# ligeroinc/ligero-prover

Measured on AMD Instinct MI355X. Metric: prover constraints/sec, higher is better.
Workload: dtype u32 limbs (BN254 Fr: 256-bit modular integers, 9x29-bit limbs in registers; SHA-256 words)

## Files before the change

### ligero-prover_amd/csrc/aes.hip

```cpp
#include "fr29.hpp"
#include "kernels.hpp"
#include <cstdlib>

namespace lig {

namespace {
struct AesTables { uint32_t te0[256]; uint8_t sbox[256]; };

uint8_t xtime_h(uint8_t x) { return (uint8_t)((x << 1) ^ ((x >> 7) * 0x1b)); }

const AesTables& host_tables() {
    static AesTables T;
    static bool ready = false;
    if (!ready) {
        uint8_t p = 1, q = 1;
        do {
            p = (uint8_t)(p ^ (p << 1) ^ ((p & 0x80) ? 0x1b : 0));
            q ^= (uint8_t)(q << 1); q ^= (uint8_t)(q << 2); q ^= (uint8_t)(q << 4);
            if (q & 0x80) q ^= 0x09;
            auto rol = [](uint8_t v, int s) { return (uint8_t)((v << s) | (v >> (8 - s))); };
            T.sbox[p] = (uint8_t)(q ^ rol(q, 1) ^ rol(q, 2) ^ rol(q, 3) ^ rol(q, 4) ^ 0x63);
        } while (p != 1);
        T.sbox[0] = 0x63;
        for (int i = 0; i < 256; i++) {
// ... 9 lines not shown
void aes256_expand_host(const uint8_t key[32], uint32_t rk[60]) {
    const AesTables& T = host_tables();
    auto subw = [&](uint32_t t) {
        return ((uint32_t)T.sbox[t >> 24] << 24) | ((uint32_t)T.sbox[(t >> 16) & 255] << 16) |
               ((uint32_t)T.sbox[(t >> 8) & 255] << 8) | T.sbox[t & 255];
    };
    for (int i = 0; i < 8; i++)
        rk[i] = ((uint32_t)key[4 * i] << 24) | ((uint32_t)key[4 * i + 1] << 16) | ((uint32_t)key[4 * i + 2] << 8) | key[4 * i + 3];
    uint8_t rcon = 1;
    for (int i = 8; i < 60; i++) {
        uint32_t t = rk[i - 1];
        if (i % 8 == 0) { t = subw((t << 8) | (t >> 24)) ^ ((uint32_t)rcon << 24); rcon = xtime_h(rcon); }
        else if (i % 8 == 4) t = subw(t);
        rk[i] = rk[i - 8] ^ t;
    }
}

__device__ uint32_t g_te[4 * 256];

__device__ __forceinline__ uint32_t x3(uint32_t a, uint32_t b, uint32_t c) { return __builtin_amdgcn_bitop3_b32(a, b, c, 0x96); }

struct TeView { const uint32_t* base; uint32_t off; };
template <int LOGR, int LAYOUT>
__device__ __forceinline__ uint32_t te_at(const TeView& tv, uint32_t table, uint32_t word, int shift) {
    if constexpr (LAYOUT == 1) {
        static_assert(LOGR == 4 || LAYOUT == 0, "entry-major layout: 16 replicas");
        const uint32_t a = __builtin_amdgcn_perm(word, tv.off, 0x0c0c0000u | ((4u + (uint32_t)(shift >> 3)) << 8));
        return *reinterpret_cast<const uint32_t*>(reinterpret_cast<const char*>(tv.base) + a + table * 64u);
    } else {
        const uint32_t idx = shift == 24 ? (word >> 24) : ((word >> shift) & 255u);
        return tv.base[((table << 8) + idx) << LOGR];
    }
}
template <int LOGR, int LAYOUT>
__device__ __forceinline__ void aes256_block(const uint32_t* __restrict__ rk, const TeView& tl, uint64_t block_index, uint32_t out[4]) {
    uint32_t s0 = rk[0], s1 = rk[1], s2 = (uint32_t)(block_index >> 32) ^ rk[2], s3 = (uint32_t)block_index ^ rk[3];
#define T_(t, w, sh) te_at<LOGR, LAYOUT>(tl, t, w, sh)
#pragma unroll
    for (int r = 1; r < 14; r++) {
        const uint32_t a0 = x3(T_(0, s0, 24), T_(1, s1, 16), T_(2, s2, 8)), a1 = x3(T_(0, s1, 24), T_(1, s2, 16), T_(2, s3, 8));
        const uint32_t a2 = x3(T_(0, s2, 24), T_(1, s3, 16), T_(2, s0, 8)), a3 = x3(T_(0, s3, 24), T_(1, s0, 16), T_(2, s1, 8));
        const uint32_t b0 = x3(a0, T_(3, s3, 0), rk[4 * r]), b1 = x3(a1, T_(3, s0, 0), rk[4 * r + 1]);
        const uint32_t b2 = x3(a2, T_(3, s1, 0), rk[4 * r + 2]), b3 = x3(a3, T_(3, s2, 0), rk[4 * r + 3]);
        s0 = b0; s1 = b1; s2 = b2; s3 = b3;
    }
    out[0] = x3(T_(2, s0, 24) & 0xff000000u, T_(3, s1, 16) & 0x00ff0000u, T_(0, s2, 8) & 0x0000ff00u) ^ (T_(1, s3, 0) & 0xffu) ^ rk[56];
    out[1] = x3(T_(2, s1, 24) & 0xff000000u, T_(3, s2, 16) & 0x00ff0000u, T_(0, s3, 8) & 0x0000ff00u) ^ (T_(1, s0, 0) & 0xffu) ^ rk[57];
    out[2] = x3(T_(2, s2, 24) & 0xff000000u, T_(3, s3, 16) & 0x00ff0000u, T_(0, s0, 8) & 0x0000ff00u) ^ (T_(1, s1, 0) & 0xffu) ^ rk[58];
    out[3] = x3(T_(2, s3, 24) & 0xff000000u, T_(3, s0, 16) & 0x00ff0000u, T_(0, s1, 8) & 0x0000ff00u) ^ (T_(1, s2, 0) & 0xffu) ^ rk[59];
#undef T_
}
template <int LOGR, int LAYOUT>
__device__ __forceinline__ TeView te_stage(uint32_t* te) {
    if constexpr (LAYOUT == 1) {
        for (uint32_t i = threadIdx.x; i < (1024u << LOGR); i += blockDim.x) te[i] = g_te[(((i >> 4) & 3u) << 8) + (i >> 6)];
        __syncthreads();
        return TeView{te, (threadIdx.x & 15u) * 4u};
    } else {
        for (uint32_t i = threadIdx.x; i < (1024u << LOGR); i += blockDim.x) te[i] = g_te[i >> LOGR];
        __syncthreads();
        return TeView{te + (threadIdx.x & ((1u << LOGR) - 1)), 0u};
    }
}
template <int LOGR, int LAYOUT>
__device__ __forceinline__ fr aes_field_elem(const uint32_t* __restrict__ rk, const TeView& tl, uint64_t elem) {
    uint32_t o[8];
    aes256_block<LOGR, LAYOUT>(rk, tl, 2 * elem, o);
    aes256_block<LOGR, LAYOUT>(rk, tl, 2 * elem + 1, o + 4);
    fr v;
#pragma unroll
    for (int i = 0; i < 8; i++) v.v[i] = __builtin_bswap32(o[i]);
#pragma unroll
    for (int i = 0; i < 8; i++) v.v[i] = (v.v[i] >> 2) | (i < 7 ? (v.v[i + 1] << 30) : 0u);
    return fr_reduce_once(v);
}

template <int LOGR, int LAYOUT = 0>
__global__ void __launch_bounds__(256) k_rng_fill(const uint32_t* __restrict__ rk, uint64_t first_elem, fr* __restrict__ out, size_t count) {
    __shared__ uint32_t te[1024 << LOGR];
    const TeView tl = te_stage<LOGR, LAYOUT>(te);
    for (size_t e = (size_t)blockIdx.x * blockDim.x + threadIdx.x; e < count; e += (size_t)gridDim.x * blockDim.x)
        fr_store(out + e, aes_field_elem<LOGR, LAYOUT>(rk, tl, first_elem + e));
}

template <int LOGR, int LAYOUT = 0>
__global__ void __launch_bounds__(256) k_rng_fill_indexed(const uint32_t* __restrict__ rk, uint64_t first_elem, const uint32_t* __restrict__ idx,
                                                          fr* __restrict__ out, size_t count) {
    __shared__ uint32_t te[1024 << LOGR];
    const TeView tl = te_stage<LOGR, LAYOUT>(te);
    for (size_t e = (size_t)blockIdx.x * blockDim.x + threadIdx.x; e < count; e += (size_t)gridDim.x * blockDim.x)
        fr_store(out + e, aes_field_elem<LOGR, LAYOUT>(rk, tl, first_elem + idx[e]));
}

template <int LOGR, int LAYOUT = 0>
__global__ void __launch_bounds__(256) k_rng_fill_rows(const uint32_t* __restrict__ rk, uint64_t first, fr* __restrict__ out, size_t rows,
                                                       uint32_t per_row, size_t row_stride, uint32_t col_off, uint32_t elem_stride, uint64_t stream_stride) {
    __shared__ uint32_t te[1024 << LOGR];
    const TeView tl = te_stage<LOGR, LAYOUT>(te);
    const size_t total = rows * per_row;
    for (size_t e = (size_t)blockIdx.x * blockDim.x + threadIdx.x; e < total; e += (size_t)gridDim.x * blockDim.x) {
        const size_t r = e / per_row;
        const uint32_t i = (uint32_t)(e - r * per_row);
        fr_store(out + r * row_stride + col_off + (size_t)i * elem_stride, aes_field_elem<LOGR, LAYOUT>(rk, tl, first + r * stream_stride + i));
    }
}
template <int LOGR, int LAYOUT = 0>
__global__ void __launch_bounds__(256) k_rng_fill_rows_dense(const uint32_t* __restrict__ rk, uint64_t first, fr* __restrict__ out, size_t rows,
                                                             uint32_t per_row, uint32_t k) {
    __shared__ uint32_t te[1024 << LOGR];
    const TeView tl = te_stage<LOGR, LAYOUT>(te);
    const size_t total = rows * k;
    for (size_t e = (size_t)blockIdx.x * blockDim.x + threadIdx.x; e < total; e += (size_t)gridDim.x * blockDim.x) {
        const size_t r = e / k;
        const uint32_t i = (uint32_t)(e - r * k);
        fr_store(out + e, i < per_row ? aes_field_elem<LOGR, LAYOUT>(rk, tl, first + r * (uint64_t)per_row + i) : fr_zero());
    }
}
#ifndef LIG_RLC_THREADS
#define LIG_RLC_THREADS 256
#endif
template <int LOGR, int LAYOUT = 0>
__global__ void __launch_bounds__(LIG_RLC_THREADS) k_rand_rlc(const uint32_t* __restrict__ rk, uint64_t first, fr* __restrict__ rand_out,
                                                  const fr* __restrict__ msgs, size_t rows, uint32_t per_row, uint32_t k,
                                                  const f29s* __restrict__ rc, uint32_t group_rows, fr* __restrict__ code_part,
                                                  fr* __restrict__ lin_part) {
    __shared__ uint32_t te[1024 << LOGR];
    const TeView tl = te_stage<LOGR, LAYOUT>(te);
    const uint32_t jblocks = k / blockDim.x, groups = (uint32_t)((rows + group_rows - 1) / group_rows), tiles = jblocks * groups;
    for (uint32_t tile = blockIdx.x; tile < tiles; tile += gridDim.x) {
        const uint32_t g = tile / jblocks, j = (tile - g * jblocks) * blockDim.x + threadIdx.x;
        const size_t r0 = (size_t)g * group_rows, r1 = r0 + group_rows < rows ? r0 + group_rows : rows;
        const bool live = j < per_row;
        f29 ac = rc != nullptr ? unpack29(fr_load(code_part + (size_t)g * k + j)) : f29_zero(), al = f29_zero();
        int since = 0;
        for (size_t r = r0; r < r1; r++) {
            const f29 u = unpack29(fr_load(msgs + r * k + j));
            if (rc != nullptr) ac = f29_add(ac, f29_montmul(u, f29_load_tab(rc + r)));
            fr v = fr_zero();
            if (live) {
                v = aes_field_elem<LOGR, LAYOUT>(rk, tl, first + r * (uint64_t)per_row + j);
                al = f29_add(al, f29_montmul(u, unpack29(v)));
            }
            fr_store(rand_out + r * k + j, v);
            if (++since == 6) { ac = f29_qnorm(ac); al = f29_qnorm(al); since = 0; }
        }
        if (rc != nullptr) fr_store(code_part + (size_t)g * k + j, pack29(f29_reduce_2p(ac)));
        f29 w = f29_montmul(f29_qnorm(al), f29_const_r2());
        w = f29_reduce_2p(f29_add(w, unpack29(fr_load(lin_part + (size_t)g * k + j))));
        fr_store(lin_part + (size_t)g * k + j, pack29(w));
    }
}

static constexpr size_t BIG_FILL = (size_t)1 << 20;
#ifndef LIG_AES_REP
#define LIG_AES_REP 4
#endif
static constexpr int REP = LIG_AES_REP;
static constexpr uint32_t BIG_BLOCKS_MAX = 256u * (REP >= 4 ? 2u : REP == 3 ? 4u : 8u);
#define BIG_BLOCKS (lig::knobs().aes_blocks ? lig::knobs().aes_blocks : BIG_BLOCKS_MAX)
#define PERM_LAYOUT (REP == 4 && lig::knobs().aes_layout == 1)
static inline uint32_t small_blocks(size_t total, size_t cap) { size_t b = (total + 255) / 256; return (uint32_t)(b > cap ? cap : b); }
void launch_rng_fill_rows_dense(hipStream_t s, const uint32_t* rk60_dev, uint64_t first, fr* out, size_t rows, uint32_t per_row, uint32_t k) {
    const size_t total = rows * k;
    if (!total) return;
    if (total >= BIG_FILL && PERM_LAYOUT) hipLaunchKernelGGL((k_rng_fill_rows_dense<4, 1>), dim3(BIG_BLOCKS), dim3(256), 0, s, rk60_dev, first, out, rows, per_row, k);
    else if (total >= BIG_FILL) hipLaunchKernelGGL(k_rng_fill_rows_dense<REP>, dim3(BIG_BLOCKS), dim3(256), 0, s, rk60_dev, first, out, rows, per_row, k);
    else hipLaunchKernelGGL(k_rng_fill_rows_dense<0>, dim3(small_blocks(total, 8192)), dim3(256), 0, s, rk60_dev, first, out, rows, per_row, k);
}

void launch_rand_rlc(hipStream_t s, const uint32_t* rk60_dev, uint64_t first, fr* out, const fr* msgs, size_t rows, uint32_t per_row, uint32_t k,
                     const f29s* rc_dev, uint32_t group_rows, fr* code_part, fr* lin_part) {
    if (!rows) return;
    const uint32_t th = (k % LIG_RLC_THREADS == 0) ? LIG_RLC_THREADS : 256;
    const size_t tiles = (size_t)(k / th) * ((rows + group_rows - 1) / group_rows);
    if (rows * k >= BIG_FILL && PERM_LAYOUT)
        hipLaunchKernelGGL((k_rand_rlc<4, 1>), dim3((uint32_t)(tiles < BIG_BLOCKS ? tiles : BIG_BLOCKS)), dim3(th), 0, s, rk60_dev, first, out, msgs, rows, per_row, k,
                           rc_dev, group_rows, code_part, lin_part);
    else if (rows * k >= BIG_FILL)
        hipLaunchKernelGGL(k_rand_rlc<REP>, dim3((uint32_t)(tiles < BIG_BLOCKS ? tiles : BIG_BLOCKS)), dim3(th), 0, s, rk60_dev, first, out, msgs, rows, per_row, k,
                           rc_dev, group_rows, code_part, lin_part);
    else
        hipLaunchKernelGGL(k_rand_rlc<0>, dim3((uint32_t)(tiles < 8192 ? tiles : 8192)), dim3(th), 0, s, rk60_dev, first, out, msgs, rows, per_row, k, rc_dev,
                           group_rows, code_part, lin_part);
}

void launch_rng_fill_rows(hipStream_t s, const uint32_t* rk60_dev, uint64_t first, fr* out, size_t rows, uint32_t per_row,
                          size_t row_stride, uint32_t col_off, uint32_t elem_stride, uint64_t stream_stride) {
    const size_t total = rows * per_row;
    if (!total) return;
    if (total >= BIG_FILL && PERM_LAYOUT)
        hipLaunchKernelGGL((k_rng_fill_rows<4, 1>), dim3(BIG_BLOCKS), dim3(256), 0, s, rk60_dev, first, out, rows, per_row, row_stride, col_off, elem_stride, stream_stride);
    else if (total >= BIG_FILL)
        hipLaunchKernelGGL(k_rng_fill_rows<REP>, dim3(BIG_BLOCKS), dim3(256), 0, s, rk60_dev, first, out, rows, per_row, row_stride, col_off, elem_stride, stream_stride);
    else
        hipLaunchKernelGGL(k_rng_fill_rows<0>, dim3(small_blocks(total, 8192)), dim3(256), 0, s, rk60_dev, first, out, rows, per_row, row_stride, col_off,
                           elem_stride, stream_stride);
}

void aes_upload_tables() {
    const AesTables& T = host_tables();
    uint32_t te[4 * 256];
    for (int t = 0; t < 4; t++)
        for (int i = 0; i < 256; i++) te[256 * t + i] = t ? (T.te0[i] >> (8 * t)) | (T.te0[i] << (32 - 8 * t)) : T.te0[i];
    (void)hipMemcpyToSymbol(HIP_SYMBOL(g_te), te, sizeof(te));
}

void launch_rng_fill(hipStream_t s, const uint32_t* rk60_dev, uint64_t first_elem, fr* out, size_t count) {
    if (!count) return;
    if (count >= BIG_FILL && PERM_LAYOUT) hipLaunchKernelGGL((k_rng_fill<4, 1>), dim3(BIG_BLOCKS), dim3(256), 0, s, rk60_dev, first_elem, out, count);
    else if (count >= BIG_FILL) hipLaunchKernelGGL(k_rng_fill<REP>, dim3(BIG_BLOCKS), dim3(256), 0, s, rk60_dev, first_elem, out, count);
    else hipLaunchKernelGGL(k_rng_fill<0>, dim3(small_blocks(count, 4096)), dim3(256), 0, s, rk60_dev, first_elem, out, count);
}

void launch_rng_fill_indexed(hipStream_t s, const uint32_t* rk60_dev, uint64_t first_elem, const uint32_t* idx_dev, fr* out, size_t count) {
    if (!count) return;
    if (count >= BIG_FILL && PERM_LAYOUT) hipLaunchKernelGGL((k_rng_fill_indexed<4, 1>), dim3(BIG_BLOCKS), dim3(256), 0, s, rk60_dev, first_elem, idx_dev, out, count);
// ... 6 lines not shown
```

### ligero-prover_amd/csrc/ctx_internal.hpp

```cpp
#pragma once
#include <hip/hip_runtime.h>
#include <functional>
#include <mutex>
#include <string>
#include <unordered_map>
#include <utility>
#include <vector>
#include "../../include/lig_hip.h"
#include "kernels.hpp"

using lig::fr;


struct lig_ctx {
    int device = 0;
    uint32_t l = 0, k = 0, n = 0;
    hipStream_t stream = nullptr;
    hipStream_t stream2 = nullptr;
    bool side_shared = false, copy_is_main = false;
    hipStream_t stream3 = nullptr;
    hipStream_t stream_sha = nullptr;
    hipEvent_t ev_fork = nullptr, ev_join = nullptr;
    lig::NttPlan plan_half;
    std::string err;
// ... 15 lines not shown
    uint32_t* tri_dev = nullptr; size_t tri_cap = 0;
    bool streams_shared = false;
    bool prof_on = false;
    std::vector<std::pair<hipEvent_t, hipEvent_t>> prof_events;
    size_t prof_used = 0;
    uint64_t prof_rows = 0;
    std::vector<uint32_t> prof_launch_rows;
    std::vector<std::pair<void*, void (*)(void*)>> comms;
    std::mutex debug_mu;
    std::function<std::string()> debug_state;
};
inline hipStream_t lig_internal_copy_stream(lig_ctx* c) {
    if (!c->stream3 && hipStreamCreateWithFlags(&c->stream3, hipStreamNonBlocking) != hipSuccess) { (void)hipGetLastError(); c->stream3 = c->stream; c->copy_is_main = true; }
    return c->stream3;
}
inline void sync_all_streams(lig_ctx* c) { for (hipStream_t st : {c->stream, c->stream2, c->stream3, c->stream_sha}) if (st) (void)hipStreamSynchronize(st); }
inline void lig_internal_set_debug_state(lig_ctx* c, std::function<std::string()> f) { std::lock_guard<std::mutex> lk(c->debug_mu); c->debug_state = std::move(f); }
inline std::string lig_internal_debug_state(lig_ctx* c) { std::lock_guard<std::mutex> lk(c->debug_mu); return c->debug_state ? c->debug_state() : std::string(); }

inline void lig_internal_comms_release(lig_ctx* c) {
    auto v = std::move(c->comms);
    c->comms.clear();
    for (auto& e : v) e.second(e.first);
}
inline void lig_internal_comm_unregister(lig_ctx* c, void* obj) {
    for (size_t i = 0; i < c->comms.size(); i++) if (c->comms[i].first == obj) { c->comms.erase(c->comms.begin() + i); return; }
}

int lig_internal_comm_fault(lig_ctx* c, bool stream_ordered);

int lig_internal_encode_rows(lig_ctx* c, const void* msgs, void* out, size_t rows, int mode, hipStream_t on = nullptr, int phases = 15,
                             void* y_scratch = nullptr, void* z_scratch = nullptr);
int lig_internal_encode_dot(lig_ctx* c, const void* rands, size_t rows, const void* cw2, size_t cw2_stride, uint32_t group_rows, void* part, hipStream_t on = nullptr,
                            bool cw2_z = false);
int lig_internal_extend_2k(lig_ctx* c, void* buf);
int lig_internal_decode_to(lig_ctx* c, const void* src, void* dst);
int lig_internal_encode_2k_rows(lig_ctx* c, void* buf, size_t rows, hipStream_t on = nullptr);
int lig_internal_encode_generic(lig_ctx* c, void* buf, hipStream_t on = nullptr);
int lig_internal_upload_small(lig_ctx* c, void* dst, const void* src, size_t bytes, hipStream_t st);
int lig_internal_download(lig_ctx* c, void* host_pinned, const void* src, size_t bytes, hipStream_t st);
int lig_internal_reserve_scratch(lig_ctx* c, size_t rows);

#define CHECK_CTX(c) do { if (!(c)) return LIG_E_ARG; if (hipSetDevice((c)->device) != hipSuccess) { (c)->err = "hipSetDevice failed"; return LIG_E_HIP; } } while (0)
#define HIP_TRY(c, call) do { hipError_t e__ = (call); if (e__ != hipSuccess) { (c)->err = std::string(#call) + ": " + hipGetErrorString(e__); return LIG_E_HIP; } } while (0)
#define FAIL(c, code, msg) do { (c)->err = (msg); return (code); } while (0)
```

### ligero-prover_amd/csrc/kernels.hpp

```cpp
#pragma once
#include <hip/hip_runtime.h>
#include <stddef.h>
#include <stdint.h>
#include <string>
#include "fr.hpp"

namespace lig {
struct Knobs {
    int      encode_kmask = 15;
    uint32_t k13_block = 256;
    uint32_t k2_dyn_lds = 0;
    size_t   encode_chunk = 512;
    bool     encode_generic = false;
    uint32_t sha_block = 256;
    int      sha_ws = 2;
    uint32_t aes_blocks = 0;
    bool     shared_side = true;
    int      aes_layout = 1;
    int      sha_gate = 1;
    size_t   sha_gate_rows = 2;
    int      sha_prio = 0;
    int      ctx_low_prio_every = 0;
    int      sha_cumask = 0;
    size_t   s1_head = 128, s1_tail = 96, s2_head = 192;
    bool     fused_rlc = true;
    bool     early_code = true;
    int      upload_mode = 2;
    bool     upload_prio = true;
    int      fault_upload = 0;
    int      upload_timeout_s = 5;
    bool     shard_uploader = false;
    int      rands_upload_mode = 2;
    bool     spin_wait = true;
    int      spin_wait_ms = 50;
    bool     d2h_kernel = true;
    bool     shard_force_exchange = false;
    bool     zres = false;
    bool     trace = false;
    int      fault_comm = 0;
    int      comm_timeout_s = 300;
    int      ipc_host_s = 120;
    int      ipc_stall_s = 120;
    std::string stream_map;
    std::string stream_pad;
    std::string rccl_lib;
};
const Knobs& knobs();
}

namespace lig {

struct NttPlan {
    uint32_t N = 0, log2N = 0;
    fr* w = nullptr;
    fr* winv = nullptr;
    fr ninv;
};
// ... 71 lines not shown
```

### ligero-prover_amd/csrc/lig_capi.hip

```cpp
#include <hip/hip_runtime.h>
#include <atomic>
#include <cstdio>
#include <cstdlib>
#include <cstring>
#include <string>
#include <unordered_map>
#include <vector>

#include <unistd.h>
#include "../../include/lig_hip.h"
#include "host_field.hpp"
#include "kernels.hpp"
#include "fr29.hpp"
#include "ctx_internal.hpp"

namespace lig {
void aes_upload_tables();
void launch_rng_fill_rows_dense(hipStream_t s, const uint32_t* rk60_dev, uint64_t first, fr* out, size_t rows, uint32_t per_row, uint32_t k);
}

namespace H = lig::host;

static fr to_dev(const H::Fr& a) {
    fr r;
// ... 229 lines not shown
            for (uint32_t j = 0; j < M / 2; j++) t[(M / 2 - 1) + j] = to_f29s(pw[(size_t)j * (S / M)]);
        t[S - 1] = to_f29s(H::from_u64(1));
        return t;
    };
    int rc;
    if ((rc = upload29(c, stage_table(H::pow_u64(w, B), A), &tp.tw_a)) != LIG_OK) return rc;
    if ((rc = upload29(c, stage_table(H::pow_u64(w, A), B), &tp.tw_b)) != LIG_OK) return rc;
    std::vector<lig::f29s> mid((size_t)N);
    const H::Fr scale = inverse ? H::inv(H::from_u64(N)) : H::from_u64(1);
    H::Fr base = H::from_u64(1);
    for (uint32_t k1 = 0; k1 < A; k1++) {
        H::Fr cur = scale;
        for (uint32_t n2 = 0; n2 < B; n2++) { mid[(size_t)k1 * B + n2] = to_f29s(cur); cur = H::mul(cur, base); }
        base = H::mul(base, w);
    }
    return upload29(c, mid, &tp.mid);
}

const lig::Knobs& lig::knobs() {
    static const lig::Knobs k = [] {
        lig::Knobs t;
        auto num = [](const char* name, long dflt) { const char* e = std::getenv(name); return e && *e ? std::atol(e) : dflt; };
        auto pos = [&](const char* name, long dflt) { const long v = num(name, 0); return v > 0 ? v : dflt; };
        t.encode_kmask = (int)num("LIG_ENCODE_KMASK", 15);
        { const long v = num("LIG_K13_BLOCK", 0); t.k13_block = (v == 64 || v == 128) ? (uint32_t)v : 256u; }
        t.k2_dyn_lds = (uint32_t)num("LIG_K2_DYN_LDS", 0);
        t.encode_chunk = (size_t)pos("LIG_ENCODE_CHUNK", 512);
        { const char* e = std::getenv("LIG_ENCODE_GENERIC"); t.encode_generic = e && e[0] == '1'; }
        t.sha_block = (uint32_t)pos("LIG_SHA_BLOCK", 256);
        { const long v = num("LIG_SHA_WS", 2); t.sha_ws = (v == 0 || v == 1 || v == 4) ? (int)v : 2; }
        t.sha_gate = (int)num("LIG_SHA_GATE", 1);
        { const long v = num("LIG_AES_BLOCKS", 0); t.aes_blocks = v >= 64 && v <= 4096 ? (uint32_t)v : 0u; }
        t.aes_layout = (int)num("LIG_AES_LAYOUT", 1);
        t.shared_side = num("LIG_SHARED_SIDE", 1) != 0;
        t.sha_gate_rows = (size_t)pos("LIG_SHA_GATE_ROWS", 2);
#ifdef LIG_EXPERIMENTS
        t.sha_prio = (int)num("LIG_SHA_PRIO", 0);
        if (const char* v = std::getenv("LIG_STREAM_MAP")) t.stream_map = v;
        if (const char* v = std::getenv("LIG_STREAM_PAD")) t.stream_pad = v;
        t.sha_cumask = (int)num("LIG_SHA_CUMASK", 0);
        t.ctx_low_prio_every = (int)num("LIG_CTX_LOW_PRIO_EVERY", 0);
#endif
        t.s1_head = (size_t)num("LIG_S1_HEAD", 128); t.s1_tail = (size_t)num("LIG_S1_TAIL", 96); t.s2_head = (size_t)num("LIG_S2_HEAD", 192);
        t.fused_rlc = std::getenv("LIG_NO_FUSED_RLC") == nullptr;
        t.early_code = num("LIG_EARLY_CODE", 1) != 0;
        t.upload_mode = (int)num("LIG_UPLOAD_MODE", 2);
        t.rands_upload_mode = (int)num("LIG_RANDS_UPLOAD_MODE", 2);
        t.upload_prio = num("LIG_UPLOAD_PRIO", 1) != 0;
        t.shard_uploader = num("LIG_SHARD_UPLOADER", 0) != 0;
        t.upload_timeout_s = (int)pos("LIG_UPLOAD_TIMEOUT_S", 5);
        t.fault_upload = (int)num("LIG_FAULT_UPLOAD", 0);
        t.d2h_kernel = num("LIG_D2H_KERNEL", 1) != 0;
        t.spin_wait = num("LIG_SPIN_WAIT", 1) != 0;
        t.spin_wait_ms = (int)pos("LIG_SPIN_WAIT_MS", 50);
        t.shard_force_exchange = std::getenv("LIG_SHARD_FORCE_EXCHANGE") != nullptr;
        t.trace = std::getenv("LIG_TRACE") != nullptr;
        t.zres = num("LIG_ZRES", 0) != 0;
        t.fault_comm = (int)num("LIG_FAULT_COMM", 0);
        t.ipc_stall_s = (int)pos("LIG_IPC_STALL_S", 120);
        t.ipc_host_s = (int)pos("LIG_IPC_HOST_S", 120);
        t.comm_timeout_s = (int)pos("LIG_COMM_TIMEOUT_S", 300);
        { const char* e = std::getenv("LIG_RCCL_LIB"); if (e) t.rccl_lib = e; }
        return t;
    }();
    return k;
}

int lig_internal_comm_fault(lig_ctx* c, bool stream_ordered) {
    const int f = lig::knobs().fault_comm;
    if (!f) return 0;
    if (f == 3 && stream_ordered) for (;;) sleep(3600);
    if ((stream_ordered && (f == 1 || f == 2)) || (!stream_ordered && f == 2)) {
        if (c) c->err = std::string("injected fault (LIG_FAULT_COMM) in the ") + (stream_ordered ? "stream-ordered" : "host-synchronous") + " all-to-all";
        return 1;
    }
// ... 306 lines not shown
            HIP_TRY(c, hipMemcpy2DAsync(z, n * sizeof(fr), (const fr*)msgs + r0 * k, k * sizeof(fr), k * sizeof(fr), nr, hipMemcpyDeviceToDevice, st));
            lig::ntt_generic_inverse(st, c->plan[LIG_SIZE_K], z, nr, n);
            lig::ntt_generic_forward(st, c->plan[LIG_SIZE_N], z, nr, n);
            for (size_t r = 0; r < nr; r++)
                for (uint32_t cs = 1; cs < 4; cs++)
                    HIP_TRY(c, hipMemcpy2DAsync((fr*)out + (r0 + r) * 3 * k + (cs - 1) * k, sizeof(fr), z + r * n + cs, 4 * sizeof(fr), sizeof(fr), k,
                                                hipMemcpyDeviceToDevice, st));
        }
    } else if (!half) {
        HIP_TRY(c, hipMemsetAsync(out, 0, rows * out_stride * sizeof(fr), st));
        HIP_TRY(c, hipMemcpy2DAsync(out, out_stride * sizeof(fr), msgs, (size_t)c->k * sizeof(fr), (size_t)c->k * sizeof(fr),
                                    rows, hipMemcpyDeviceToDevice, st));
        lig::ntt_generic_inverse(st, c->plan[LIG_SIZE_K], (fr*)out, rows, out_stride);
        lig::ntt_generic_forward(st, c->plan[LIG_SIZE_N], (fr*)out, rows, out_stride);
    } else {
        const size_t k2 = 2 * (size_t)c->k, chunk = 64;
        int rc = ensure_scratch(c, rows < chunk ? rows : chunk);
        if (rc != LIG_OK) return rc;
        for (size_t r0 = 0; r0 < rows; r0 += chunk) {
            const size_t nr = rows - r0 < chunk ? rows - r0 : chunk;
            fr* z = c->scratch_z;
            HIP_TRY(c, hipMemsetAsync(z, 0, nr * k2 * sizeof(fr), st));
            HIP_TRY(c, hipMemcpy2DAsync(z, k2 * sizeof(fr), (const fr*)msgs + r0 * c->k, (size_t)c->k * sizeof(fr), (size_t)c->k * sizeof(fr),
                                        nr, hipMemcpyDeviceToDevice, st));
            lig::ntt_generic_inverse(st, c->plan[LIG_SIZE_K], z, nr, k2);
            lig::ntt_generic_forward(st, c->plan_half, z, nr, k2);
            HIP_TRY(c, hipMemcpy2DAsync((fr*)out + r0 * c->k, sizeof(fr), z + 1, 2 * sizeof(fr), sizeof(fr), nr * (size_t)c->k,
                                        hipMemcpyDeviceToDevice, st));
        }
    }
    HIP_TRY(c, hipGetLastError());
    return LIG_OK;
}
int lig_internal_encode_dot(lig_ctx* c, const void* rands, size_t rows, const void* cw2, size_t cw2_stride, uint32_t group_rows, void* part, hipStream_t on, bool cw2_z) {
    if (!c->fast) return LIG_E_STATE;
    hipStream_t st = on ? on : c->stream;
    int rc = ensure_scratch(c, rows);
    if (rc != LIG_OK) return rc;
    const lig::EncodeDot dot{(const fr*)cw2, cw2_stride, group_rows, (fr*)part, cw2_z};
    lig::encode_rows_fast(st, c->ep, (const fr*)rands, nullptr, c->scratch_y, c->scratch_z, rows, nullptr, nullptr, lig::ENC_DOT, &dot);
    HIP_TRY(c, hipGetLastError());
    return LIG_OK;
}
static fr* tiled_scratch_for(lig_ctx* c, hipStream_t st) { return c->tiled_scratch[st == c->stream2 ? 1 : 0]; }

int lig_internal_encode_2k_rows(lig_ctx* c, void* buf, size_t rows, hipStream_t on) {
    hipStream_t st = on ? on : c->stream;
    if (c->tiled && rows <= 3) {
        lig::ntt_tiled(st, c->tplan[LIG_SIZE_2K][1], (fr*)buf, c->n, (fr*)buf, c->n, rows, tiled_scratch_for(c, st));
        lig::ntt_tiled(st, c->tplan[LIG_SIZE_N][0], (fr*)buf, c->n, (fr*)buf, c->n, rows, tiled_scratch_for(c, st));
        HIP_TRY(c, hipGetLastError());
        return LIG_OK;
    }
    lig::ntt_generic_inverse(st, c->plan[LIG_SIZE_2K], (fr*)buf, rows, c->n);
    lig::ntt_generic_forward(st, c->plan[LIG_SIZE_N], (fr*)buf, rows, c->n);
    HIP_TRY(c, hipGetLastError());
    return LIG_OK;
}
int lig_internal_encode_generic(lig_ctx* c, void* buf, hipStream_t on) {
    hipStream_t st = on ? on : c->stream;
    if (c->tiled) {
        lig::ntt_tiled(st, c->tplan[LIG_SIZE_K][1], (fr*)buf, c->n, (fr*)buf, c->n, 1, tiled_scratch_for(c, st));
        lig::ntt_tiled(st, c->tplan[LIG_SIZE_N][0], (fr*)buf, c->n, (fr*)buf, c->n, 1, tiled_scratch_for(c, st));
        HIP_TRY(c, hipGetLastError());
        return LIG_OK;
    }
    lig::ntt_generic_inverse(st, c->plan[LIG_SIZE_K], (fr*)buf, 1, c->n);
    lig::ntt_generic_forward(st, c->plan[LIG_SIZE_N], (fr*)buf, 1, c->n);
    HIP_TRY(c, hipGetLastError());
    return LIG_OK;
}
int lig_internal_decode_to(lig_ctx* c, const void* src, void* dst) {
    if (c->tiled) {
// ... 301 lines not shown
```

### ligero-prover_amd/csrc/prover.hip

```cpp
#include "prover_common.hpp"
#include "upload.hpp"
#include <cerrno>
#include <functional>

struct lig_trace {
    lig_ctx* c = nullptr;
    lig_synth_job job;
    bool from_rows = false;
    bool loaded = false, committed = false;
    bool dense_rands = false;
    bool diag_ok = false;
    fr* msgs_alt = nullptr;
    bool alt_pending = false;
    JobHeader hdr;
    std::vector<RowDesc> rows;
    std::vector<PadRun> pad_runs;
    uint64_t mask_pos = 0;
    std::vector<std::pair<size_t, size_t>> sched1;
    const uint8_t* host_msgs = nullptr;
    std::vector<hipEvent_t> ev_up;
    FlagPage flags;
    UploadLane up, rand;
    bool up_by_thread = false;
    fr* rands_full = nullptr;
// ... 329 lines not shown
struct RandSource { const fr* dev = nullptr; const uint8_t* host = nullptr; bool pushed = false;
                    lig_linear* linear = nullptr; };

static int prove_stage23(lig_trace* T, const RandSource& rs, const uint8_t* const_sum_given, const uint8_t** proof, size_t* proof_len,
                         lig_proof_info* info, const std::function<void(const char*)>& mark) {
    lig_ctx* c = T->c;
    const uint32_t l = c->l, k = c->k, n = c->n, t = 192;
    const size_t R = T->R;
    hipStream_t s = c->stream, s2 = c->stream2;
    auto t0 = clk::now();
    uint32_t rk[60];
    const size_t NT = T->triples.size() / 3;
    lig::aes256_expand_host(info->stage1_seed, rk);
    TRY(lig_internal_upload_small(c, c->rk_dev, rk, sizeof rk, s));
    fr* code = T->acc; fr* lin = T->acc + n; fr* quad = T->acc + 2 * (size_t)n; fr* tmp = T->acc + 3 * (size_t)n;
    fr* linH = lin + 2 * (size_t)k; fr* linC = lin + 3 * (size_t)k;
    const size_t groups = (lig_tune::CHUNK + lig_tune::GROUP - 1) / lig_tune::GROUP;
    fr* p_code = T->parts; fr* p_linH = T->parts + groups * (size_t)n; fr* p_linC = T->parts + 2 * groups * (size_t)n;
    const size_t dot_groups = (lig_tune::CHUNK + lig_tune::DOT_GROUP - 1) / lig_tune::DOT_GROUP;
    HIP_TRY(c, hipMemsetAsync(T->parts, 0, (2 * groups * (size_t)n + dot_groups * k) * 32, s));
    HIP_TRY(c, hipMemsetAsync(T->acc, 0, 4 * (size_t)n * 32, s));
    fr* rhalf = T->rcw;
    const size_t s2_head = lig::knobs().s2_head;
    const std::vector<std::pair<size_t, size_t>> sched2 = chunk_schedule(R, lig_tune::CHUNK, s2_head, 0);
    const size_t n_chunks = sched2.size();
    std::vector<uint64_t> chunk_pos(n_chunks + 1, 0);
    for (size_t ci = 0; ci < n_chunks; ci++) {
        uint64_t cnt = 0;
        for (size_t r = sched2[ci].first; r < sched2[ci].second; r++) cnt += T->rows[r].data;
        chunk_pos[ci + 1] = chunk_pos[ci] + cnt;
    }
    auto rand_buf = [&](size_t ci) -> fr* { return rs.dev ? const_cast<fr*>(rs.dev) + sched2[ci].first * (size_t)k : T->randb + (ci & 1) * lig_tune::CHUNK * (size_t)k; };
    const bool fused_rlc = !rs.dev && !rs.host && (k % 256 == 0) && lig::knobs().fused_rlc;
    const bool early_code = lig::knobs().early_code;
    const lig::f29s* rc_loop = early_code ? nullptr : T->coef_dev;
    const bool rands_by_thread = rs.host && lig::knobs().upload_mode == 2 && lig::knobs().rands_upload_mode == 2 && lig_internal_uploader_available(c) && n_chunks;
    uint32_t rseq = 0;
    const lig::FlagLayout fl = T->flag_layout(n_chunks);
    if (rands_by_thread) {
        TRY(T->flags.ensure(c, fl.words));
        if (fl.consumed + n_chunks > fl.words) FAIL(c, LIG_E_STATE, "rows job: flag page too small for the stage-2 schedule");
        rseq = ++T->rand.seq;
        T->up_abort.store(0, std::memory_order_release);
        std::vector<lig::UploadChunk> chunks;
        for (size_t ci = 0; ci < n_chunks; ci++) chunks.push_back({(uint8_t*)rand_buf(ci), rs.host + sched2[ci].first * (size_t)k * 32, (sched2[ci].second - sched2[ci].first) * (size_t)k * 32});
        lig_internal_uploader_submit(c->device, lig::chunk_jobs(chunks, T->flags.host + fl.rands, rseq, &T->rand.failed, T->flags.host + fl.consumed, &T->up_abort, 1), &T->rand.pending);
    }
    auto form_rand_chunk = [&](size_t ci) -> int {
        const size_t b = sched2[ci].first, nb = sched2[ci].second - sched2[ci].first;
        fr* rb = rand_buf(ci);
        if (rs.pushed) return LIG_OK;
        if (rs.dev) { HIP_TRY(c, hipEventRecord(T->ev_ready[ci & 1], s2)); return LIG_OK; }
        if (rands_by_thread) return LIG_OK;
        if (ci >= 2) HIP_TRY(c, hipStreamWaitEvent(s2, T->ev_used[ci & 1], 0));
        if (rs.host) {
            HIP_TRY(c, hipMemcpyAsync(rb, rs.host + b * (size_t)k * 32, nb * (size_t)k * 32, hipMemcpyHostToDevice, s2));
        } else {
            uint64_t lpos = chunk_pos[ci];
            for (size_t r = 0; r < nb;) {
                size_t run = 1;
                const uint32_t d = T->rows[b + r].data;
                while (r + run < nb && T->rows[b + r + run].data == d) run++;
                if (fused_rlc) lig::launch_rand_rlc(s2, c->rk_dev, lpos, rb + r * k, T->msgs + (b + r) * k, run, d, k, rc_loop ? rc_loop + b + r : nullptr, lig_tune::GROUP / 4, p_code, p_linH);
                else lig::launch_rng_fill_rows_dense(s2, c->rk_dev, lpos, rb + r * k, run, d, k);
                lpos += (uint64_t)run * d; r += run;
            }
// ... 1 lines not shown
        HIP_TRY(c, hipEventRecord(T->ev_ready[ci & 1], s2));
        return LIG_OK;
    };
    {
        const std::vector<lig::f29s> coef = coef_table(draw_coefficients(info->stage1_seed, T->rows), nullptr, nullptr);
        TRY(lig_internal_upload_small(c, T->coef_dev, coef.data(), coef.size() * sizeof(lig::f29s), s));
    }
    HIP_TRY(c, hipEventRecord(c->ev_fork, s));
    HIP_TRY(c, hipStreamWaitEvent(s2, c->ev_fork, 0));
    if (rs.linear) TRY(lig_internal_linear_form(c, rs.linear, c->rk_dev, const_cast<fr*>(rs.dev), s2));
    if (n_chunks) TRY(form_rand_chunk(0));
    fr* mask = T->maskcw; fr* mlin = mask + n; fr* mquad = mask + 2 * (size_t)n;
    uint8_t* enc = T->h_enc;
    const size_t vec_bytes = (size_t)n * 32;
    if (early_code) {
        for (size_t b = 0; b < R; b += lig_tune::CHUNK) {
            const size_t nb = std::min<size_t>(lig_tune::CHUNK, R - b);
            lig::launch_rlc_accumulate29(s, T->msgs + b * k, k, 1, nullptr, 0, nb, k, T->coef_dev + b, p_code, nullptr, lig_tune::GROUP / 4);
        }
        lig::launch_rlc_combine(s, tmp, p_code, (uint32_t)((lig_tune::CHUNK + lig_tune::GROUP / 4 - 1) / (lig_tune::GROUP / 4)), k);
        TRY(lig_internal_encode_rows(c, tmp, code, 1, false));
        lig::launch_eltwise(s, LIG_OP_ADD_ASSIGN, mask, nullptr, code, n, fr{}, 0);
        TRY(lig_internal_download(c, enc, code, vec_bytes, s));
        HIP_TRY(c, hipEventRecord(T->ev_acc[0], s));
    }
    for (size_t ci = 0; ci < n_chunks; ci++) {
        const size_t b = sched2[ci].first, nb = sched2[ci].second - sched2[ci].first;
        fr* rb = rand_buf(ci);
        if (ci + 1 < n_chunks) TRY(form_rand_chunk(ci + 1));
        if (rs.pushed && !T->push_sync) HIP_TRY(c, hipStreamWaitValue32(s, T->flags.dev + fl.push, (uint32_t)sched2[ci].second, hipStreamWaitValueGte, 0xffffffffu));
        else if (rands_by_thread) HIP_TRY(c, hipStreamWaitValue32(s, T->flags.dev + fl.rands + ci, rseq, hipStreamWaitValueGte, 0xffffffffu));
        else HIP_TRY(c, hipStreamWaitEvent(s, T->ev_ready[ci & 1], 0));
        if (c->fast) {
            TRY(lig_internal_encode_dot(c, rb, nb, T->cw + b * 3 * (size_t)k + k, 3 * (size_t)k, lig_tune::DOT_GROUP, p_linC, nullptr, T->zres));
        } else {
            TRY(lig_internal_encode_rows(c, rb, rhalf, nb, lig::ENC_HALF));
            lig::launch_rlc_accumulate29(s, T->cw + b * 3 * (size_t)k + k, 3 * (size_t)k, 1, rhalf, k, nb, k, nullptr, nullptr, p_linC, lig_tune::DOT_GROUP);
        }
        if (!fused_rlc) lig::launch_rlc_accumulate29(s, T->msgs + b * k, k, 1, rb, k, nb, k, rc_loop ? rc_loop + b : nullptr, p_code, p_linH, lig_tune::GROUP / 4);
        if (rands_by_thread) HIP_TRY(c, hipStreamWriteValue32(s, T->flags.dev + fl.consumed + ci, rseq, 0));
        else HIP_TRY(c, hipEventRecord(T->ev_used[ci & 1], s));
    }
    {
        const uint32_t pg = (uint32_t)((lig_tune::CHUNK + lig_tune::GROUP / 4 - 1) / (lig_tune::GROUP / 4));
        if (!early_code) lig::launch_rlc_combine(s, tmp, p_code, pg, k);
        lig::launch_rlc_combine(s, linH, p_linH, pg, k);
        lig::launch_rlc_combine(s, linC, p_linC, (uint32_t)dot_groups, k);
    }
    mark("stage2 rows (rng+dot+encode+rlc)");
    lig::launch_sum_elems(s, linH, k, 1, T->dots, nullptr);
    lig::launch_lin_interleave(s, lin, linH, linC, k);
    HIP_TRY(c, hipMemsetAsync(lin + 2 * (size_t)k, 0, (size_t)(n - 2 * k) * 32, s));
    const lig::CwView view{T->msgs, T->cw, k};
    lig::launch_quad_rows29_view(s, view, 2 * k, T->tri_dev, T->coef_dev + R, T->coef_dev + R + NT, NT, quad, T->parts, 2 * groups * (size_t)n);
    const H::Fr* dots = reinterpret_cast<const H::Fr*>(T->h_small);
    TRY(lig_internal_download(c, T->h_small, T->dots, 32, s));
    if (!early_code) {
        TRY(lig_internal_encode_rows(c, tmp, code, 1, false));
        lig::launch_eltwise(s, LIG_OP_ADD_ASSIGN, mask, nullptr, code, n, fr{}, 0);
        TRY(lig_internal_download(c, enc, code, vec_bytes, s));
        HIP_TRY(c, hipEventRecord(T->ev_acc[0], s));
    }
    TRY(lig_internal_extend_2k(c, lin));
    lig::launch_eltwise(s, LIG_OP_ADD_ASSIGN, mlin, nullptr, lin, n, fr{}, 0);
    TRY(lig_internal_download(c, enc + vec_bytes, lin, vec_bytes, s));
    HIP_TRY(c, hipEventRecord(T->ev_acc[1], s));
    TRY(lig_internal_extend_2k(c, quad));
    lig::launch_eltwise(s, LIG_OP_ADD_ASSIGN, mquad, nullptr, quad, n, fr{}, 0);
    TRY(lig_internal_download(c, enc + 2 * vec_bytes, quad, vec_bytes, s));
    HIP_TRY(c, hipEventRecord(T->ev_acc[2], s));
    H::Fr* dec = reinterpret_cast<H::Fr*>(T->h_small + 32);
    const fr* accs[3] = {code, lin, quad};
    for (int a3 = 0; a3 < 3; a3++) {
        TRY(lig_internal_decode_to(c, accs[a3], tmp));
// ... 512 lines not shown
```

Before: 2.080 billion.

## Hoist counter-independent AES first rounds into per-block head and share across block pair

Precomputes the parts of the first AES round that depend only on the key and the constant words s0/s1, storing them as wave-uniform scalars. It also evaluates the two counter blocks of each field element jointly, since they differ only in the low bit of s3, so most of rounds 1-2 are computed once and shared. This cuts table lookups in the RNG-fused kernels. It also adds env knobs for the RLC block size and for recording the rand-buffer-free event earlier, after the encode tiles; both default off.

```diff
diff --git a/ligero-prover_amd/csrc/aes.hip b/ligero-prover_amd/csrc/aes.hip
--- a/ligero-prover_amd/csrc/aes.hip
+++ b/ligero-prover_amd/csrc/aes.hip
@@ -65,12 +65,22 @@
         return tv.base[((table << 8) + idx) << LOGR];
     }
 }
-template <int LOGR, int LAYOUT>
-__device__ __forceinline__ void aes256_block(const uint32_t* __restrict__ rk, const TeView& tl, uint64_t block_index, uint32_t out[4]) {
-    uint32_t s0 = rk[0], s1 = rk[1], s2 = (uint32_t)(block_index >> 32) ^ rk[2], s3 = (uint32_t)block_index ^ rk[3];
+struct AesHead { uint32_t c0, c1, c2, c3; };
 #define T_(t, w, sh) te_at<LOGR, LAYOUT>(tl, t, w, sh)
+template <int LOGR, int LAYOUT>
+__device__ __forceinline__ AesHead aes_head(const uint32_t* __restrict__ rk, const TeView& tl) {
+    const uint32_t s0 = rk[0], s1 = rk[1];
+    AesHead h;
+    h.c0 = __builtin_amdgcn_readfirstlane(x3(T_(0, s0, 24), T_(1, s1, 16), rk[4]));
+    h.c1 = __builtin_amdgcn_readfirstlane(x3(T_(0, s1, 24), T_(3, s0, 0), rk[5]));
+    h.c2 = __builtin_amdgcn_readfirstlane(x3(T_(2, s0, 8), T_(3, s1, 0), rk[6]));
+    h.c3 = __builtin_amdgcn_readfirstlane(x3(T_(1, s0, 16), T_(2, s1, 8), rk[7]));
+    return h;
+}
+template <int LOGR, int LAYOUT, int R0>
+__device__ __forceinline__ void aes256_tail(const uint32_t* __restrict__ rk, const TeView& tl, uint32_t s0, uint32_t s1, uint32_t s2, uint32_t s3, uint32_t out[4]) {
 #pragma unroll
-    for (int r = 1; r < 14; r++) {
+    for (int r = R0; r < 14; r++) {
         const uint32_t a0 = x3(T_(0, s0, 24), T_(1, s1, 16), T_(2, s2, 8)), a1 = x3(T_(0, s1, 24), T_(1, s2, 16), T_(2, s3, 8));
         const uint32_t a2 = x3(T_(0, s2, 24), T_(1, s3, 16), T_(2, s0, 8)), a3 = x3(T_(0, s3, 24), T_(1, s0, 16), T_(2, s1, 8));
         const uint32_t b0 = x3(a0, T_(3, s3, 0), rk[4 * r]), b1 = x3(a1, T_(3, s0, 0), rk[4 * r + 1]);
@@ -81,8 +91,19 @@
     out[1] = x3(T_(2, s1, 24) & 0xff000000u, T_(3, s2, 16) & 0x00ff0000u, T_(0, s3, 8) & 0x0000ff00u) ^ (T_(1, s0, 0) & 0xffu) ^ rk[57];
     out[2] = x3(T_(2, s2, 24) & 0xff000000u, T_(3, s3, 16) & 0x00ff0000u, T_(0, s0, 8) & 0x0000ff00u) ^ (T_(1, s1, 0) & 0xffu) ^ rk[58];
     out[3] = x3(T_(2, s3, 24) & 0xff000000u, T_(3, s0, 16) & 0x00ff0000u, T_(0, s1, 8) & 0x0000ff00u) ^ (T_(1, s2, 0) & 0xffu) ^ rk[59];
+}
+template <int LOGR, int LAYOUT>
+__device__ __forceinline__ void aes256_block_pair(const uint32_t* __restrict__ rk, const TeView& tl, const AesHead& h, uint64_t even_block, uint32_t out[8]) {
+    const uint32_t s2 = (uint32_t)(even_block >> 32) ^ rk[2], s3 = (uint32_t)even_block ^ rk[3], s3o = s3 ^ 1u;
+    const uint32_t t2 = T_(2, s2, 8);
+    const uint32_t e0 = x3(t2, T_(3, s3, 0), h.c0), o0 = x3(t2, T_(3, s3o, 0), h.c0);
+    const uint32_t w1 = x3(T_(1, s2, 16), T_(2, s3, 8), h.c1), w2 = x3(T_(0, s2, 24), T_(1, s3, 16), h.c2), w3 = x3(T_(0, s3, 24), T_(3, s2, 0), h.c3);
+    const uint32_t p0 = x3(T_(1, w1, 16), T_(2, w2, 8), T_(3, w3, 0)), p1 = x3(T_(0, w1, 24), T_(1, w2, 16), T_(2, w3, 8));
+    const uint32_t p2 = x3(T_(0, w2, 24), T_(1, w3, 16), T_(3, w1, 0)), p3 = x3(T_(0, w3, 24), T_(2, w1, 8), T_(3, w2, 0));
+    aes256_tail<LOGR, LAYOUT, 3>(rk, tl, x3(p0, T_(0, e0, 24), rk[8]), x3(p1, T_(3, e0, 0), rk[9]), x3(p2, T_(2, e0, 8), rk[10]), x3(p3, T_(1, e0, 16), rk[11]), out);
+    aes256_tail<LOGR, LAYOUT, 3>(rk, tl, x3(p0, T_(0, o0, 24), rk[8]), x3(p1, T_(3, o0, 0), rk[9]), x3(p2, T_(2, o0, 8), rk[10]), x3(p3, T_(1, o0, 16), rk[11]), out + 4);
+}
 #undef T_
-}
 template <int LOGR, int LAYOUT>
 __device__ __forceinline__ TeView te_stage(uint32_t* te) {
     if constexpr (LAYOUT == 1) {
@@ -96,10 +117,9 @@
     }
 }
 template <int LOGR, int LAYOUT>
-__device__ __forceinline__ fr aes_field_elem(const uint32_t* __restrict__ rk, const TeView& tl, uint64_t elem) {
+__device__ __forceinline__ fr aes_field_elem(const uint32_t* __restrict__ rk, const TeView& tl, const AesHead& h, uint64_t elem) {
     uint32_t o[8];
-    aes256_block<LOGR, LAYOUT>(rk, tl, 2 * elem, o);
-    aes256_block<LOGR, LAYOUT>(rk, tl, 2 * elem + 1, o + 4);
+    aes256_block_pair<LOGR, LAYOUT>(rk, tl, h, 2 * elem, o);
     fr v;
 #pragma unroll
     for (int i = 0; i < 8; i++) v.v[i] = __builtin_bswap32(o[i]);
@@ -112,8 +132,9 @@
 __global__ void __launch_bounds__(256) k_rng_fill(const uint32_t* __restrict__ rk, uint64_t first_elem, fr* __restrict__ out, size_t count) {
     __shared__ uint32_t te[1024 << LOGR];
     const TeView tl = te_stage<LOGR, LAYOUT>(te);
+    const AesHead hd = aes_head<LOGR, LAYOUT>(rk, tl);
     for (size_t e = (size_t)blockIdx.x * blockDim.x + threadIdx.x; e < count; e += (size_t)gridDim.x * blockDim.x)
-        fr_store(out + e, aes_field_elem<LOGR, LAYOUT>(rk, tl, first_elem + e));
+        fr_store(out + e, aes_field_elem<LOGR, LAYOUT>(rk, tl, hd, first_elem + e));
 }
 
 template <int LOGR, int LAYOUT = 0>
@@ -121,8 +142,9 @@
                                                           fr* __restrict__ out, size_t count) {
     __shared__ uint32_t te[1024 << LOGR];
     const TeView tl = te_stage<LOGR, LAYOUT>(te);
+    const AesHead hd = aes_head<LOGR, LAYOUT>(rk, tl);
     for (size_t e = (size_t)blockIdx.x * blockDim.x + threadIdx.x; e < count; e += (size_t)gridDim.x * blockDim.x)
-        fr_store(out + e, aes_field_elem<LOGR, LAYOUT>(rk, tl, first_elem + idx[e]));
+        fr_store(out + e, aes_field_elem<LOGR, LAYOUT>(rk, tl, hd, first_elem + idx[e]));
 }
 
 template <int LOGR, int LAYOUT = 0>
@@ -130,11 +152,12 @@
                                                        uint32_t per_row, size_t row_stride, uint32_t col_off, uint32_t elem_stride, uint64_t stream_stride) {
     __shared__ uint32_t te[1024 << LOGR];
     const TeView tl = te_stage<LOGR, LAYOUT>(te);
+    const AesHead hd = aes_head<LOGR, LAYOUT>(rk, tl);
     const size_t total = rows * per_row;
     for (size_t e = (size_t)blockIdx.x * blockDim.x + threadIdx.x; e < total; e += (size_t)gridDim.x * blockDim.x) {
         const size_t r = e / per_row;
         const uint32_t i = (uint32_t)(e - r * per_row);
-        fr_store(out + r * row_stride + col_off + (size_t)i * elem_stride, aes_field_elem<LOGR, LAYOUT>(rk, tl, first + r * stream_stride + i));
+        fr_store(out + r * row_stride + col_off + (size_t)i * elem_stride, aes_field_elem<LOGR, LAYOUT>(rk, tl, hd, first + r * stream_stride + i));
     }
 }
 template <int LOGR, int LAYOUT = 0>
@@ -142,26 +165,25 @@
                                                              uint32_t per_row, uint32_t k) {
     __shared__ uint32_t te[1024 << LOGR];
     const TeView tl = te_stage<LOGR, LAYOUT>(te);
+    const AesHead hd = aes_head<LOGR, LAYOUT>(rk, tl);
     const size_t total = rows * k;
     for (size_t e = (size_t)blockIdx.x * blockDim.x + threadIdx.x; e < total; e += (size_t)gridDim.x * blockDim.x) {
         const size_t r = e / k;
         const uint32_t i = (uint32_t)(e - r * k);
-        fr_store(out + e, i < per_row ? aes_field_elem<LOGR, LAYOUT>(rk, tl, first + r * (uint64_t)per_row + i) : fr_zero());
-    }
-}
-#ifndef LIG_RLC_THREADS
-#define LIG_RLC_THREADS 256
-#endif
-template <int LOGR, int LAYOUT = 0>
-__global__ void __launch_bounds__(LIG_RLC_THREADS) k_rand_rlc(const uint32_t* __restrict__ rk, uint64_t first, fr* __restrict__ rand_out,
+        fr_store(out + e, i < per_row ? aes_field_elem<LOGR, LAYOUT>(rk, tl, hd, first + r * (uint64_t)per_row + i) : fr_zero());
+    }
+}
+template <int LOGR, int LAYOUT = 0, int THREADS = 256>
+__global__ void __launch_bounds__(THREADS) k_rand_rlc(const uint32_t* __restrict__ rk, uint64_t first, fr* __restrict__ rand_out,
                                                   const fr* __restrict__ msgs, size_t rows, uint32_t per_row, uint32_t k,
                                                   const f29s* __restrict__ rc, uint32_t group_rows, fr* __restrict__ code_part,
                                                   fr* __restrict__ lin_part) {
     __shared__ uint32_t te[1024 << LOGR];
     const TeView tl = te_stage<LOGR, LAYOUT>(te);
-    const uint32_t jblocks = k / blockDim.x, groups = (uint32_t)((rows + group_rows - 1) / group_rows), tiles = jblocks * groups;
+    const AesHead hd = aes_head<LOGR, LAYOUT>(rk, tl);
+    const uint32_t jblocks = k / THREADS, groups = (uint32_t)((rows + group_rows - 1) / group_rows), tiles = jblocks * groups;
     for (uint32_t tile = blockIdx.x; tile < tiles; tile += gridDim.x) {
-        const uint32_t g = tile / jblocks, j = (tile - g * jblocks) * blockDim.x + threadIdx.x;
+        const uint32_t g = tile / jblocks, j = (tile - g * jblocks) * THREADS + threadIdx.x;
         const size_t r0 = (size_t)g * group_rows, r1 = r0 + group_rows < rows ? r0 + group_rows : rows;
         const bool live = j < per_row;
         f29 ac = rc != nullptr ? unpack29(fr_load(code_part + (size_t)g * k + j)) : f29_zero(), al = f29_zero();
@@ -171,7 +193,7 @@
             if (rc != nullptr) ac = f29_add(ac, f29_montmul(u, f29_load_tab(rc + r)));
             fr v = fr_zero();
             if (live) {
-                v = aes_field_elem<LOGR, LAYOUT>(rk, tl, first + r * (uint64_t)per_row + j);
+                v = aes_field_elem<LOGR, LAYOUT>(rk, tl, hd, first + r * (uint64_t)per_row + j);
                 al = f29_add(al, f29_montmul(u, unpack29(v)));
             }
             fr_store(rand_out + r * k + j, v);
@@ -201,20 +223,29 @@
     else hipLaunchKernelGGL(k_rng_fill_rows_dense<0>, dim3(small_blocks(total, 8192)), dim3(256), 0, s, rk60_dev, first, out, rows, per_row, k);
 }
 
+template <int LOGR, int LAYOUT, int THREADS>
+static void launch_rand_rlc_big(hipStream_t s, const uint32_t* rk60_dev, uint64_t first, fr* out, const fr* msgs, size_t rows, uint32_t per_row, uint32_t k,
+                                const f29s* rc_dev, uint32_t group_rows, fr* code_part, fr* lin_part) {
+    const size_t tiles = (size_t)(k / THREADS) * ((rows + group_rows - 1) / group_rows);
+    const uint32_t blocks = lig::knobs().aes_blocks ? lig::knobs().aes_blocks : THREADS == 256 ? BIG_BLOCKS_MAX : 256u;
+    hipLaunchKernelGGL((k_rand_rlc<LOGR, LAYOUT, THREADS>), dim3((uint32_t)(tiles < blocks ? tiles : blocks)), dim3(THREADS), 0, s, rk60_dev, first, out, msgs, rows,
+                       per_row, k, rc_dev, group_rows, code_part, lin_part);
+}
 void launch_rand_rlc(hipStream_t s, const uint32_t* rk60_dev, uint64_t first, fr* out, const fr* msgs, size_t rows, uint32_t per_row, uint32_t k,
                      const f29s* rc_dev, uint32_t group_rows, fr* code_part, fr* lin_part) {
     if (!rows) return;
-    const uint32_t th = (k % LIG_RLC_THREADS == 0) ? LIG_RLC_THREADS : 256;
-    const size_t tiles = (size_t)(k / th) * ((rows + group_rows - 1) / group_rows);
-    if (rows * k >= BIG_FILL && PERM_LAYOUT)
-        hipLaunchKernelGGL((k_rand_rlc<4, 1>), dim3((uint32_t)(tiles < BIG_BLOCKS ? tiles : BIG_BLOCKS)), dim3(th), 0, s, rk60_dev, first, out, msgs, rows, per_row, k,
-                           rc_dev, group_rows, code_part, lin_part);
-    else if (rows * k >= BIG_FILL)
-        hipLaunchKernelGGL(k_rand_rlc<REP>, dim3((uint32_t)(tiles < BIG_BLOCKS ? tiles : BIG_BLOCKS)), dim3(th), 0, s, rk60_dev, first, out, msgs, rows, per_row, k,
-                           rc_dev, group_rows, code_part, lin_part);
-    else
-        hipLaunchKernelGGL(k_rand_rlc<0>, dim3((uint32_t)(tiles < 8192 ? tiles : 8192)), dim3(th), 0, s, rk60_dev, first, out, msgs, rows, per_row, k, rc_dev,
+    if (rows * k < BIG_FILL) {
+        const size_t tiles = (size_t)(k / 256) * ((rows + group_rows - 1) / group_rows);
+        hipLaunchKernelGGL(k_rand_rlc<0>, dim3((uint32_t)(tiles < 8192 ? tiles : 8192)), dim3(256), 0, s, rk60_dev, first, out, msgs, rows, per_row, k, rc_dev,
                            group_rows, code_part, lin_part);
+        return;
+    }
+    const uint32_t want = lig::knobs().rlc_threads, th = k % want == 0 ? want : 256;
+#define BIG_(T) (PERM_LAYOUT ? launch_rand_rlc_big<4, 1, T> : launch_rand_rlc_big<REP, 0, T>)(s, rk60_dev, first, out, msgs, rows, per_row, k, rc_dev, group_rows, code_part, lin_part)
+    if (th == 1024) BIG_(1024);
+    else if (th == 512) BIG_(512);
+    else BIG_(256);
+#undef BIG_
 }
 
 void launch_rng_fill_rows(hipStream_t s, const uint32_t* rk60_dev, uint64_t first, fr* out, size_t rows, uint32_t per_row,
diff --git a/ligero-prover_amd/csrc/ctx_internal.hpp b/ligero-prover_amd/csrc/ctx_internal.hpp
--- a/ligero-prover_amd/csrc/ctx_internal.hpp
+++ b/ligero-prover_amd/csrc/ctx_internal.hpp
@@ -71,7 +71,7 @@
 int lig_internal_encode_rows(lig_ctx* c, const void* msgs, void* out, size_t rows, int mode, hipStream_t on = nullptr, int phases = 15,
                              void* y_scratch = nullptr, void* z_scratch = nullptr);
 int lig_internal_encode_dot(lig_ctx* c, const void* rands, size_t rows, const void* cw2, size_t cw2_stride, uint32_t group_rows, void* part, hipStream_t on = nullptr,
-                            bool cw2_z = false);
+                            bool cw2_z = false, hipEvent_t after_tiles = nullptr);
 int lig_internal_extend_2k(lig_ctx* c, void* buf);
 int lig_internal_decode_to(lig_ctx* c, const void* src, void* dst);
 int lig_internal_encode_2k_rows(lig_ctx* c, void* buf, size_t rows, hipStream_t on = nullptr);
diff --git a/ligero-prover_amd/csrc/kernels.hpp b/ligero-prover_amd/csrc/kernels.hpp
--- a/ligero-prover_amd/csrc/kernels.hpp
+++ b/ligero-prover_amd/csrc/kernels.hpp
@@ -15,6 +15,7 @@
     uint32_t sha_block = 256;
     int      sha_ws = 2;
     uint32_t aes_blocks = 0;
+    uint32_t rlc_threads = 256;
     bool     shared_side = true;
     int      aes_layout = 1;
     int      sha_gate = 1;
@@ -23,6 +24,7 @@
     int      ctx_low_prio_every = 0;
     int      sha_cumask = 0;
     size_t   s1_head = 128, s1_tail = 96, s2_head = 192;
+    bool     s2_early_free = false;
     bool     fused_rlc = true;
     bool     early_code = true;
     int      upload_mode = 2;
diff --git a/ligero-prover_amd/csrc/lig_capi.hip b/ligero-prover_amd/csrc/lig_capi.hip
--- a/ligero-prover_amd/csrc/lig_capi.hip
+++ b/ligero-prover_amd/csrc/lig_capi.hip
@@ -285,6 +285,7 @@
         t.sha_gate = (int)num("LIG_SHA_GATE", 1);
         { const long v = num("LIG_AES_BLOCKS", 0); t.aes_blocks = v >= 64 && v <= 4096 ? (uint32_t)v : 0u; }
         t.aes_layout = (int)num("LIG_AES_LAYOUT", 1);
+        { const long v = num("LIG_RLC_THREADS", 0); t.rlc_threads = (v == 512 || v == 1024) ? (uint32_t)v : 256u; }
         t.shared_side = num("LIG_SHARED_SIDE", 1) != 0;
         t.sha_gate_rows = (size_t)pos("LIG_SHA_GATE_ROWS", 2);
 #ifdef LIG_EXPERIMENTS
@@ -294,6 +295,7 @@
         t.sha_cumask = (int)num("LIG_SHA_CUMASK", 0);
         t.ctx_low_prio_every = (int)num("LIG_CTX_LOW_PRIO_EVERY", 0);
 #endif
+        t.s2_early_free = num("LIG_S2_EARLY_FREE", 0) != 0;
         t.s1_head = (size_t)num("LIG_S1_HEAD", 128); t.s1_tail = (size_t)num("LIG_S1_TAIL", 96); t.s2_head = (size_t)num("LIG_S2_HEAD", 192);
         t.fused_rlc = std::getenv("LIG_NO_FUSED_RLC") == nullptr;
         t.early_code = num("LIG_EARLY_CODE", 1) != 0;
@@ -666,13 +668,13 @@
     HIP_TRY(c, hipGetLastError());
     return LIG_OK;
 }
-int lig_internal_encode_dot(lig_ctx* c, const void* rands, size_t rows, const void* cw2, size_t cw2_stride, uint32_t group_rows, void* part, hipStream_t on, bool cw2_z) {
+int lig_internal_encode_dot(lig_ctx* c, const void* rands, size_t rows, const void* cw2, size_t cw2_stride, uint32_t group_rows, void* part, hipStream_t on, bool cw2_z, hipEvent_t after_tiles) {
     if (!c->fast) return LIG_E_STATE;
     hipStream_t st = on ? on : c->stream;
     int rc = ensure_scratch(c, rows);
     if (rc != LIG_OK) return rc;
     const lig::EncodeDot dot{(const fr*)cw2, cw2_stride, group_rows, (fr*)part, cw2_z};
-    lig::encode_rows_fast(st, c->ep, (const fr*)rands, nullptr, c->scratch_y, c->scratch_z, rows, nullptr, nullptr, lig::ENC_DOT, &dot);
+    lig::encode_rows_fast(st, c->ep, (const fr*)rands, nullptr, c->scratch_y, c->scratch_z, rows, nullptr, after_tiles, lig::ENC_DOT, &dot);
     HIP_TRY(c, hipGetLastError());
     return LIG_OK;
 }
diff --git a/ligero-prover_amd/csrc/prover.hip b/ligero-prover_amd/csrc/prover.hip
--- a/ligero-prover_amd/csrc/prover.hip
+++ b/ligero-prover_amd/csrc/prover.hip
@@ -385,6 +385,7 @@
     }
     auto rand_buf = [&](size_t ci) -> fr* { return rs.dev ? const_cast<fr*>(rs.dev) + sched2[ci].first * (size_t)k : T->randb + (ci & 1) * lig_tune::CHUNK * (size_t)k; };
     const bool fused_rlc = !rs.dev && !rs.host && (k % 256 == 0) && lig::knobs().fused_rlc;
+    const bool early_free = fused_rlc && c->fast && lig::knobs().s2_early_free;
     const bool early_code = lig::knobs().early_code;
     const lig::f29s* rc_loop = early_code ? nullptr : T->coef_dev;
     const bool rands_by_thread = rs.host && lig::knobs().upload_mode == 2 && lig::knobs().rands_upload_mode == 2 && lig_internal_uploader_available(c) && n_chunks;
@@ -452,14 +453,14 @@
         else if (rands_by_thread) HIP_TRY(c, hipStreamWaitValue32(s, T->flags.dev + fl.rands + ci, rseq, hipStreamWaitValueGte, 0xffffffffu));
         else HIP_TRY(c, hipStreamWaitEvent(s, T->ev_ready[ci & 1], 0));
         if (c->fast) {
-            TRY(lig_internal_encode_dot(c, rb, nb, T->cw + b * 3 * (size_t)k + k, 3 * (size_t)k, lig_tune::DOT_GROUP, p_linC, nullptr, T->zres));
+            TRY(lig_internal_encode_dot(c, rb, nb, T->cw + b * 3 * (size_t)k + k, 3 * (size_t)k, lig_tune::DOT_GROUP, p_linC, nullptr, T->zres, early_free ? T->ev_used[ci & 1] : nullptr));
         } else {
             TRY(lig_internal_encode_rows(c, rb, rhalf, nb, lig::ENC_HALF));
             lig::launch_rlc_accumulate29(s, T->cw + b * 3 * (size_t)k + k, 3 * (size_t)k, 1, rhalf, k, nb, k, nullptr, nullptr, p_linC, lig_tune::DOT_GROUP);
         }
         if (!fused_rlc) lig::launch_rlc_accumulate29(s, T->msgs + b * k, k, 1, rb, k, nb, k, rc_loop ? rc_loop + b : nullptr, p_code, p_linH, lig_tune::GROUP / 4);
         if (rands_by_thread) HIP_TRY(c, hipStreamWriteValue32(s, T->flags.dev + fl.consumed + ci, rseq, 0));
-        else HIP_TRY(c, hipEventRecord(T->ev_used[ci & 1], s));
+        else if (!early_free) HIP_TRY(c, hipEventRecord(T->ev_used[ci & 1], s));
     }
     {
         const uint32_t pg = (uint32_t)((lig_tune::CHUNK + lig_tune::GROUP / 4 - 1) / (lig_tune::GROUP / 4));
```

After: 2.079 billion. Within noise of the previous version (-0.0%).
